# srisarya/nanopore-barcoding-ORC

Measured on AMD Instinct MI355X. Metric: Mreads/s two-round SP5×SP27 demux; % HBM roofline; 1/2/4/8 GPU, higher is better.
Workload: dtype u64

## Files before the change

nanopore-barcoding-orc_amd/csrc/dmx_device.h:

```cpp
#pragma once
#include <hip/hip_runtime.h>
#include <stdint.h>

namespace dmx {

constexpr int kMaxAdapters = 64;
constexpr int kMaxLen = 64;
constexpr int kRingSmall = 74;
constexpr int kRingLarge = 128;
constexpr int kScanBlock = 256;
constexpr int kResolveBlock = 64;

enum : uint8_t { kFront = 1, kBack = 2 };

struct DevAdapter {
    uint64_t peq[8];
    int8_t acc[72];
    int8_t pacc[72];
    uint8_t m;
    uint8_t k;
    uint8_t where;
    int8_t kk;
    uint8_t pad[4];
};
// ... 90 lines not shown

struct FTask {
    uint32_t item;
    uint32_t p0;
    uint16_t span;
    uint8_t hoff;
    uint8_t flags;
    uint32_t n, start, len;
    uint64_t off;
};
static_assert(sizeof(FTask) == 32, "FTask layout");

constexpr int kSuperNt = 4096;
constexpr int kCellGuardWords = 4;
constexpr int kCandStageCap = 128;

template <typename Rec, int CAP = kStageCap>
struct Stage {
    Rec* buf;
    uint32_t* cnt;
    uint32_t* base;
    Rec* g;
    uint32_t* gcount;
    uint32_t gcap;
    uint32_t* flags;
    uint32_t ovf;

    __device__ __forceinline__ void push(const Rec& r) const {
        const uint32_t i = atomicAdd(cnt, 1u);
        if (i < (uint32_t)CAP) {
            buf[i] = r;
            return;
        }
        const uint32_t gi = atomicAdd(gcount, 1u);
        if (gi < gcap) g[gi] = r;
        else atomicOr(flags, ovf);
    }
    __device__ __forceinline__ void flush() const {
        __syncthreads();
        const uint32_t n = min(*cnt, (uint32_t)CAP);
        if (threadIdx.x == 0) *base = n ? atomicAdd(gcount, n) : 0u;
        __syncthreads();
        const uint32_t b = *base;
        for (uint32_t i = threadIdx.x; i < n; i += blockDim.x) {
            if (b + i < gcap) g[b + i] = buf[i];
            else atomicOr(flags, ovf);
        }
        __syncthreads();
        if (threadIdx.x == 0) *cnt = 0;
        __syncthreads();
    }
};

__device__ __forceinline__ uint32_t stage_count(const uint32_t* c) {
    __syncthreads();
    const uint32_t v = *c;
    __syncthreads();
    return v;
}

struct ItemView {
    uint32_t read;
    uint32_t start;
    uint32_t len;
    uint8_t strand;
    uint8_t pad;
    int16_t only_adapter;
};

struct Cluster {
    uint32_t item;
    uint16_t sub;
    uint8_t lastcol;
    int8_t ub;
    uint32_t j1, j2;
};

struct Cand {
    uint32_t item;
    uint16_t sub;
    uint8_t iend;
    uint8_t cost;
    uint32_t j;
    uint32_t n, start, len;
    uint8_t strand, o, a, clean;
    uint64_t off;
};
static_assert(sizeof(Cand) == 40 && offsetof(Cand, off) == 32, "Cand layout");

struct Outcome {
    uint64_t key;
    int32_t origin;
    int32_t pad;
};

__host__ __device__ inline uint64_t make_key(int score, int o, int cost, int a, uint64_t t) {
    const int s = score < -128 ? -128 : score;
    return ((uint64_t)(127 - s) << 56) | ((uint64_t)o << 55) | ((uint64_t)cost << 48) |
           ((uint64_t)a << 40) | (t & ((1ull << 40) - 1));
}
__host__ __device__ inline int key_score(uint64_t k) { return 127 - (int)(k >> 56); }
__host__ __device__ inline int key_orient(uint64_t k) { return (int)((k >> 55) & 1); }
__host__ __device__ inline int key_cost(uint64_t k) { return (int)((k >> 48) & 127); }
__host__ __device__ inline int key_adapter(uint64_t k) { return (int)((k >> 40) & 255); }
__host__ __device__ inline uint64_t key_t(uint64_t k) { return k & ((1ull << 40) - 1); }

constexpr int kKeyPosBits = 40;
constexpr int kKeyDeltaBits = 4;
constexpr int kKeyDeltaBias = 8;
constexpr int kKeyDeltaMin = -kKeyDeltaBias;
constexpr int kBandMaxCost = 7;
static_assert(sizeof(uint32_t) * 8 + 1 <= kKeyPosBits - kKeyDeltaBits,
              "t = len + 1 + iend < 2^33 must fit above the delta code");
static_assert(kBandMaxCost < kKeyDeltaBias && kBandMaxCost + kKeyDeltaBias < (1 << kKeyDeltaBits),
              "|delta| <= cost <= 7 must fit the delta code");
__host__ __device__ inline uint64_t make_key_o(int score, int o, int cost, int a, uint64_t t,
                                               int delta) {
    return make_key(score, o, cost, a,
                    (t << kKeyDeltaBits) |
                        (uint64_t)((delta + kKeyDeltaBias) & ((1 << kKeyDeltaBits) - 1)));
}
__host__ __device__ inline uint64_t key_t_o(uint64_t k) { return key_t(k) >> kKeyDeltaBits; }
__host__ __device__ inline int key_delta(uint64_t k) {
    return (int)(k & ((1u << kKeyDeltaBits) - 1)) - kKeyDeltaBias;
}

enum EndType : uint8_t { kEndPrefix = 0, kEndFrontX = 1, kEndSuffix = 2, kEndBackX = 3 };
struct EndAdapter {
    uint64_t peq[4];
    int8_t acc[72];
    int8_t pacc[72];
    uint8_t m, k, type, orig;
    int8_t kk;
    uint8_t pad[3];
};
static_assert(sizeof(EndAdapter) == 184, "EndAdapter layout");
struct DevEnds {
    int32_t n;
    int32_t n_orient;
    int32_t n_sub;
    int32_t remap_on;
    uint8_t remap[kMaxAdapters];
    EndAdapter ad[kMaxAdapters];
};

enum BoundsBuf : uint32_t {
    kBufSeq = 1, kBufMask = 2, kBufSlot = 3, kBufItem = 4, kBufRes = 5, kBufCount = 6,
    kBufRead = 7, kBufLinked = 8, kBufCand = 9, kBufChop = 10, kBufPd = 11,
    kBufPaTrace = 12, kBufPaOps = 13, kBufGaCols = 14, kBufRdCols = 15, kBufRrCols = 16,
    kBufHistBins = 17, kBufRaCols = 18, kBufRaTable = 19, kBufRaBest = 20,
    kBufEndsSeq = 21, kBufEndsMask = 22, kBufEndsSlot = 23, kBufEndsItem = 24, kBufEndsRead = 25
};
enum BoundsKernel : int32_t {
    kKerFilter = 1, kKerVerify, kKerScreen, kKerScreen4, kKerWscan, kKerScan, kKerBand0,
    kKerBand1, kKerResolve, kKerSelect, kKerFin0, kKerFin1, kKerFin0L, kKerFin1L,
    kKerFin2L, kKerChop, kKerChopBig, kKerChopStart, kKerSelfTest, kKerPieces, kKerPairdist,
    kKerPairalign, kKerPairalignTb, kKerGroupalign, kKerGroupalignTb, kKerGroupalignMerge,
    kKerRowdist, kKerRowpair, kKerRowpairRc, kKerHithist, kKerRowassign,
    kKerRowassignDecide, kKerRowassignFinish, kKerEnds, kKerEndsOrigin, kKerEndsRemap,
    kKerChopViews
};
constexpr int kBoundsRec = 24;

struct Bounds {
#ifdef DMX_DEBUG_BOUNDS
    int64_t lo, hi;
    uint64_t slots, items, reads, counts, linked;
    uint64_t res, views, srcs;
    uint32_t* rec;
    int32_t kid;
#endif
};

__device__ __forceinline__ bool bchk(const Bounds& b, int64_t i, int64_t lo, int64_t hi,
                                     uint32_t buf) {
#ifdef DMX_DEBUG_BOUNDS
    if (i >= lo && i < hi) return true;
    atomicOr(b.rec + 3, 32u);
    if (atomicCAS(b.rec + kBoundsRec, 0u, (uint32_t)b.kid + 1u) == 0u) {
        b.rec[kBoundsRec + 1] = buf;
        b.rec[kBoundsRec + 2] = (uint32_t)(uint64_t)i;
        b.rec[kBoundsRec + 3] = (uint32_t)((uint64_t)i >> 32);
    }
    return false;
#else
    (void)b, (void)i, (void)lo, (void)hi, (void)buf;
    return true;
#endif
}
#ifdef DMX_DEBUG_BOUNDS
#define DMX_BOUND(bd, field, i, buf) bchk((bd), (int64_t)(i), 0, (int64_t)(bd).field, (buf))
#else
#define DMX_BOUND(bd, field, i, buf) true
#endif

constexpr int kGuardWords = 64;
constexpr int kGuardNt = 16 * kGuardWords;
constexpr int kMinOffset = 16;
constexpr int kMinTail = 64;
constexpr int kViewReachPre = 64;

struct Packed {
    const uint32_t* seq;
    const uint32_t* nmask;
    Bounds bd;
};
constexpr int kOffBits = 36;
constexpr uint64_t kOffMask = (1ull << kOffBits) - 1ull;

__device__ __forceinline__ uint32_t window32(const uint32_t* __restrict__ w, int64_t bitpos,
                                             const Bounds& bd, uint32_t buf) {
    const int64_t q = bitpos >> 5;
    const uint32_t sh = (uint32_t)bitpos & 31u;
#ifdef DMX_DEBUG_BOUNDS
    if (!bchk(bd, q, bd.lo, bd.hi - 1, buf)) return 0u;
#else
    (void)bd, (void)buf;
#endif
    uint64_t v;
    __builtin_memcpy(&v, w + q, 8);
    return (uint32_t)(v >> sh);
}
__device__ __forceinline__ uint32_t code32(const Packed& pk, int64_t g) {
    return window32(pk.seq, 2 * g, pk.bd, kBufSeq);
}
__device__ __forceinline__ uint32_t mask32(const Packed& pk, int64_t g) {
    return window32(pk.nmask, g, pk.bd, kBufMask);
}

__device__ __forceinline__ uint32_t rev_pairs(uint32_t w) {
    const uint32_t v = __brev(w);
    return ((v >> 1) & 0x55555555u) | ((v << 1) & 0xAAAAAAAAu);
}

__device__ __forceinline__ void fetch16(const Packed& pk, uint64_t off, uint32_t n,
                                        uint32_t strand, uint32_t start, uint32_t p,
                                        uint32_t& codes, uint32_t& nbits, bool load_mask = true) {
    if (strand == 0) {
        const int64_t g = (int64_t)off + start + p;
        codes = code32(pk, g);
        nbits = load_mask ? mask32(pk, g) & 0xFFFFu : 0u;
    } else {
        const int64_t b = (int64_t)off + (int64_t)n - 1 - start - (int64_t)p - 15;
        codes = ~rev_pairs(code32(pk, b));
        nbits = load_mask ? __brev(mask32(pk, b)) >> 16 : 0u;
    }
}

template <int HB>
__device__ __forceinline__ void myers_step_hw(uint32_t eql, uint32_t eqh, uint32_t& pvl,
                                              uint32_t& pvh, uint32_t& mvl, uint32_t& mvh, int& d,
                                              uint32_t hbit) {
    const uint32_t xvl = eql | mvl, xvh = eqh | mvh;
    uint32_t cy, cy2;
    const uint32_t sl = __builtin_addc(eql & pvl, pvl, 0u, &cy);
    const uint32_t sh = __builtin_addc(eqh & pvh, pvh, cy, &cy2);
    const uint32_t xhl = (sl ^ pvl) | eql, xhh = (sh ^ pvh) | eqh;
    const uint32_t phl = mvl | ~(xhl | pvl), phh = mvh | ~(xhh | pvh);
    const uint32_t mhl = pvl & xhl, mhh = pvh & xhh;
    uint32_t ps, ms;
    if constexpr (HB == 0) {
        ps = phl;
        ms = mhl;
    } else if constexpr (HB == 1) {
        ps = phh;
        ms = mhh;
    } else {
        ps = hbit >= 32 ? phh : phl;
        ms = hbit >= 32 ? mhh : mhl;
    }
    d += (int)__builtin_amdgcn_ubfe(ps, hbit & 31u, 1) +
         __builtin_amdgcn_sbfe((int)ms, hbit & 31u, 1);
    const uint32_t phh1 = __builtin_amdgcn_alignbit(phh, phl, 31), phl1 = phl << 1;
    const uint32_t mhh1 = __builtin_amdgcn_alignbit(mhh, mhl, 31), mhl1 = mhl << 1;
    pvl = mhl1 | ~(xvl | phl1);
    pvh = mhh1 | ~(xvh | phh1);
    mvl = phl1 & xvl;
    mvh = phh1 & xvh;
}

template <int HB = -1>
__device__ __forceinline__ void myers_step(uint64_t eq, uint64_t& pv, uint64_t& mv, int& d,
                                           uint32_t hbit) {
    uint32_t pvl = (uint32_t)pv, pvh = (uint32_t)(pv >> 32);
    uint32_t mvl = (uint32_t)mv, mvh = (uint32_t)(mv >> 32);
    myers_step_hw<HB>((uint32_t)eq, (uint32_t)(eq >> 32), pvl, pvh, mvl, mvh, d, hbit);
    pv = ((uint64_t)pvh << 32) | pvl;
    mv = ((uint64_t)mvh << 32) | mvl;
}

__device__ __forceinline__ void myers_step32(uint32_t eq, uint32_t& pv, uint32_t& mv, int& d,
                                             uint32_t hbit) {
    const uint32_t xv = eq | mv;
    const uint32_t xh = (((eq & pv) + pv) ^ pv) | eq;
    uint32_t ph = mv | ~(xh | pv);
    uint32_t mh = pv & xh;
    d += (int)__builtin_amdgcn_ubfe(ph, hbit, 1) + __builtin_amdgcn_sbfe((int)mh, hbit, 1);
    ph <<= 1;
    mh <<= 1;
    pv = mh | ~(xv | ph);
    mv = ph & xv;
}

__device__ __forceinline__ int col_cost(uint64_t pv, uint64_t mv, int i) {
    const uint64_t mask = i >= 64 ? ~0ull : ((1ull << i) - 1ull);
    return __popcll(pv & mask) - __popcll(mv & mask);
}

}
```

nanopore-barcoding-orc_amd/csrc/dmx_kernels.hip:

```cpp
#include <algorithm>
#include <cstring>
#include <memory>
#include <type_traits>
#include <utility>
#include <vector>

#include "dmx_device.h"
#include "dmx_internal.h"

namespace dmx {

struct RoundArgs {
    Packed pk;
    const uint64_t* offs;
    const uint32_t* lens;
    const DevPanel* panel;
    const ItemView* items;
    const uint32_t* n_items_dev;
    uint32_t n_items;
    int32_t T;
    int32_t per_task_slot;
    int32_t slot_div;
    Cluster* cl;
    Outcome* outc;
// ... 1753 lines not shown
                const bool reached = ps_emit(R, fbuf, fcnt, rr, item, o, tvo);
                ps_lastcol(R, wbuf, wcnt, last && !reached, item, o, tvo, rb);
            }
        }
    }
}

constexpr int kSbWords = kSuperNt / 16 + 8;

typedef __attribute__((address_space(1))) uint32_t gu32;
struct CellPtrs {
    gu32* p[4];
    __device__ __forceinline__ explicit CellPtrs(const RoundArgs& R) {
#pragma unroll
        for (int i = 0; i < 4; ++i) p[i] = sgpr_ptr(R.cells[i]);
    }
};

__device__ __forceinline__ void flat_check(const RoundArgs& R, const CellPtrs& cp,
                                           const PsTables& tb, uint64_t cw, uint64_t X,
                                           bool valid) {
    gu32* p1 = nullptr;
    uint32_t b1 = 0;
    if (valid) {
        const uint32_t kr = ps_key(tb, (uint32_t)(cw >> 6) & 0xFFFFu);
        const int64_t last = (int64_t)R.n_words * 16 - 1;
        const int e0 = (int)(kr & 0xFFFFu), e1 = e0 + (int)(kr >> 16);
        for (int e = e0; e < e1; ++e) {
            const uint64_t ev = tb.ent[e];
            const int len = (int)((ev >> 32) & 31u);
            const int off = (int)((ev >> 38) & 3u);
            const uint32_t msk = len >= 16 ? ~0u : ((1u << (2 * len)) - 1u);
            if (((uint32_t)(cw >> (2 * (3 - off))) & msk) != (uint32_t)ev) continue;
            const int tau = (int)((ev >> 37) & 1u);
            const int dlo = (int)((ev >> 40) & 255u) - 128;
            const int dhi = (int)((ev >> 48) & 255u) - 128;
            const int64_t x = (int64_t)X - off;
            int64_t nlo = tau ? x - dhi : x + len + dlo - 1;
            int64_t nhi = tau ? x - dlo : x + len + dhi - 1;
            nlo = nlo < 0 ? 0 : nlo;
            nhi = nhi > last ? last : nhi;
            if (nlo > nhi) continue;
            const int ci = 2 * (int)((ev >> 56) & 1u) + tau;
            gu32* cells = ci < 2 ? (ci == 0 ? cp.p[0] : cp.p[1]) : (ci == 2 ? cp.p[2] : cp.p[3]);
            for (int64_t c = nlo >> 4; c <= (nhi >> 4);) {
                const int64_t w = c >> 5;
                const int64_t cend = min(nhi >> 4, (w << 5) + 31);
                const uint32_t bits = (uint32_t)((((2ull << (cend - c)) - 1ull)) << (c & 31));
                if (!p1) {
                    p1 = cells + w;
                    b1 = bits;
                } else {
                    __hip_atomic_fetch_or(cells + w, bits, __ATOMIC_RELAXED, __HIP_MEMORY_SCOPE_AGENT);
                }
                c = cend + 1;
            }
        }
    }
    const uint64_t pa = (uint64_t)p1;
    const uint64_t pl = ((uint64_t)__shfl_up((uint32_t)(pa >> 32), 1u, 64) << 32) |
                        (uint64_t)__shfl_up((uint32_t)pa, 1u, 64);
    const uint32_t bl = __shfl_up(b1, 1u, 64);
    const bool dup = (threadIdx.x & 63u) != 0u && pl == pa && (bl & b1) == b1;
    if (p1 && !dup) {
        __hip_atomic_fetch_or(p1, b1, __ATOMIC_RELAXED, __HIP_MEMORY_SCOPE_AGENT);
    }
}

template <int S>
__global__ __launch_bounds__(kPScanBlock) void pscan_kernel(RoundArgs R) {
    static_assert(S == 1 || S == 2 || S == 4, "sampling stride: 64 positions per step");
    extern __shared__ __attribute__((aligned(16))) uint8_t s_dyn[];
    __shared__ __attribute__((aligned(16))) uint32_t s_sb[kPScanBlock / 64][kSbWords];
    __shared__ uint16_t s_q[kPScanBlock / 64][64];
    const PsTables tb = ps_load_tables(R.pieces, s_dyn);
    __syncthreads();
    const CellPtrs cp(R);
    const int lane = (int)(threadIdx.x & 63u);
    uint32_t* const sbw = s_sb[threadIdx.x >> 6];
    uint16_t* const q = s_q[threadIdx.x >> 6];
    const uint4* sp = reinterpret_cast<const uint4*>(R.pk.seq);
    const uint32_t nw = gridDim.x * (kPScanBlock / 64);
    for (uint32_t sb = blockIdx.x * (kPScanBlock / 64) + (threadIdx.x >> 6); sb < R.nsb; sb += nw) {
        const int64_t wd = (int64_t)sb * (kSuperNt / 16) + 4 * lane;
        const bool live = wd < (int64_t)R.n_words;
        uint4 c = {0u, 0u, 0u, 0u};
        if (live) c = sp[wd >> 2];
        uint32_t w0 = __shfl_up(c.w, 1u, 64), w5 = __shfl_down(c.x, 1u, 64);
        if (lane == 0) w0 = R.pk.seq[wd - 1];
        if (lane == 63) w5 = live ? R.pk.seq[wd + 4] : 0u;
        auto hits = ps_lookups<S>(tb.pr, w0, c.x, c.y, c.z, c.w, w5);
        using HitT = decltype(hits);
        if (!live) hits = 0;
        reinterpret_cast<uint4*>(sbw)[1 + lane] = c;
        if (lane == 0) sbw[3] = w0;
        if (lane == 63) {
            sbw[kSbWords - 4] = w5;
            sbw[kSbWords - 3] = 0u;
            sbw[kSbWords - 2] = 0u;
            sbw[kSbWords - 1] = 0u;
        }
        uint32_t total;
        uint32_t idx = wave_excl_scan((uint32_t)__popcll((unsigned long long)hits), total);
        const uint64_t C0 = (uint64_t)sb * kSuperNt;
        for (uint32_t base = 0; base < total; base += 64) {
            while (hits && idx < base + 64u) {
                const int qq = (int)__builtin_ctzll((unsigned long long)hits);
                hits &= hits - (HitT)1;
                q[idx - base] = (uint16_t)(lane * 64 + qq * S);
                ++idx;
            }
            __builtin_amdgcn_wave_barrier();
            const bool v = (uint32_t)lane < total - base;
            const uint32_t p = v ? q[lane] : 0u;
            const uint32_t t = p + 61u;
            const uint32_t wi = t >> 4, sh = 2u * (t & 15u);
            const uint64_t lo = ((uint64_t)sbw[wi + 1] << 32) | sbw[wi];
            const uint64_t cw = sh ? (lo >> sh) | ((uint64_t)sbw[wi + 2] << (64u - sh)) : lo;
            flat_check(R, cp, tb, cw, C0 + p, v);
            __builtin_amdgcn_wave_barrier();
        }
    }
}

__global__ __launch_bounds__(kScanBlock) void pcompact_kernel(RoundArgs R) {
    const DevPanel* P = R.panel;
    const DevPieces* Q = R.pieces;
    const uint32_t n_items = R.items ? *R.n_items_dev : R.n_items;
    const bool front = P->where == kFront;
    const int A = P->n_adapters;
    const int no = P->n_orient;
    const int W = P->scan_len + P->kf;
    const int SEG = kSegSpan - W;
    const int rb = kCleanHist ? P->clean_reach : 0;
    const int fr = Q->front_reach;
    const uint32_t wsh = wave_shard();
    FTask* const fbuf = R.ftask + wsh * R.ftask_scap;
    uint32_t* const fcnt = R.ftask_count + wsh * kShardStride;
    Window* const wbuf = R.win + wsh * R.win_scap;
    uint32_t* const wcnt = R.win_count + wsh * kShardStride;
    const uint32_t stride = gridDim.x * blockDim.x;
    const CellPtrs cp(R);
    const gu32* const cb0 = cp.p[2 * R.round];
    const gu32* const cb1 = cp.p[2 * R.round + 1];
    struct View {
        TaskView tv;
        int64_t p0nt = 0;
        int delta = 0, ncell = 0, l = 0;
        uint3 w = {0u, 0u, 0u};
    };
    const auto words = [&](const View& v, int k0, uint3& wv) __attribute__((always_inline)) {
        const int64_t c0 = v.p0nt >> 4;
        const int64_t cs = v.tv.strand ? c0 - k0 - 63 : c0 + k0;
        const gu32* cb = v.tv.strand ? cb1 : cb0;
        const int64_t w = k0 < v.ncell ? cs >> 5 : 0;
        wv.x = cb[w];
        wv.y = cb[w + 1];
        wv.z = cb[w + 2];
    };
    const auto prep = [&](uint32_t item, bool act, int o, View& v) __attribute__((always_inline)) {
        if (act) {
            task_view(R, item, o * A, A, v.tv);
            v.l = (int)v.tv.len;
        }
        v.p0nt = v.tv.strand ? (int64_t)v.tv.off + v.tv.n - 1 - v.tv.start
                             : (int64_t)v.tv.off + v.tv.start;
        v.delta = act ? (v.tv.strand ? 15 - (int)(v.p0nt & 15) : (int)(v.p0nt & 15)) : 0;
        v.ncell = act && v.l > 0 ? (v.l + v.delta + 15) >> 4 : 0;
        words(v, 0, v.w);
    };
    const auto run = [&](uint32_t item, bool act, int o, const View& v) __attribute__((always_inline)) {
        bool reached = false;
        uint3 cur = v.w;
        for (int k0 = 0; __ballot(k0 < v.ncell); k0 += 64) {
            uint3 nx = {0u, 0u, 0u};
            words(v, k0 + 64, nx);
            uint64_t m = 0;
            if (k0 < v.ncell) {
                const int64_t c0 = v.p0nt >> 4;
                const int64_t cs = v.tv.strand ? c0 - k0 - 63 : c0 + k0;
                const uint32_t sh = (uint32_t)(cs & 31);
                const uint64_t lo = ((uint64_t)cur.y << 32) | cur.x;
                const uint64_t x = sh ? (lo >> sh) | ((uint64_t)cur.z << (64 - sh)) : lo;
                m = v.tv.strand ? __builtin_bitreverse64(x) : x;
                if (front && k0 == 0)
                    m |= (fr + v.delta + 15) >> 4 >= 64 ? ~0ull
                                                        : ((1ull << ((fr + v.delta + 15) >> 4)) - 1ull);
                const int left = v.ncell - k0;
                if (left < 64) m &= (1ull << left) - 1ull;
                m |= ((m << 1) & (m >> 1)) | ((m << 1) & (m >> 2)) | ((m << 2) & (m >> 1));
            }
            PsRuns rr{m, k0, v.delta, v.l, W, SEG, 0, 0};
            reached |= ps_emit(R, fbuf, fcnt, rr, item, o, v.tv);
            cur = nx;
        }
        ps_lastcol(R, wbuf, wcnt, act && !front && !reached, item, o, v.tv, rb);
    };
    for (uint32_t i0 = blockIdx.x * blockDim.x; i0 < n_items; i0 += stride) {
        const uint32_t item = i0 + threadIdx.x;
        const bool act = item < n_items;
        View v0, v1;
        v0.tv.strand = v1.tv.strand = 0;
        const bool act1 = act && no > 1;
        prep(item, act, 0, v0);
        prep(item, act1, 1, v1);
        run(item, act, 0, v0);
        run(item, act1, 1, v1);
    }
}

__global__ __launch_bounds__(kScanBlock) __attribute__((amdgpu_waves_per_eu(DMX_FILTER_WAVES))) void ftask_kernel(RoundArgs R) {
    __shared__ uint32_t s_fpeq[8];
    __shared__ __attribute__((aligned(16))) int8_t s_thr[kScanBlock];
    __shared__ Window s_win[kScanBlock / 64][kWaveWinCap];
    __shared__ uint32_t s_wcnt[kScanBlock / 64];
    __shared__ uint32_t s_spre[kShards + 1];
    const DevPanel* P = R.panel;
    const int L = P->scan_len;
    const int kf = P->kf;
    if (threadIdx.x < 8) s_fpeq[threadIdx.x] = P->filter_peq[threadIdx.x];
    if (threadIdx.x < kScanBlock / 64) s_wcnt[threadIdx.x] = 0;
    {
        const int far0 = min((int)P->kf, (int)P->pf[71]);
        const int j = (int)threadIdx.x + 1;
        int t = -1;
        for (int d = 0; d <= far0; ++d)
            if (d <= (int)P->pf[min(j + d, 71)]) t = d;
        s_thr[threadIdx.x] = (int8_t)t;
    }
    ShardMap sm{s_spre, 0u};
    sm.load(R.ftask_count, R.ftask_scap);
    const uint32_t total = sm.total();
    const uint32_t wv = threadIdx.x >> 6;
    const uint32_t wsh = wave_shard();
    const WaveStage<Window, kWaveWinCap> st{s_win[wv], &s_wcnt[wv], R.win + wsh * R.win_scap,
                                            R.win_count + wsh * kShardStride, R.win_scap,
                                            R.flags, 4u};
    const bool front = P->where == kFront;
    const int kf_far = min(kf, (int)P->pf[71]);
    const uint32_t gap = (uint32_t)P->max_mk;
    const int rb = kCleanHist ? P->clean_reach : 0;
    const uint32_t pv_rows = L >= 32 ? ~0u : ~0u << (32 - L);
    for (uint32_t tb = blockIdx.x * kScanBlock; tb < total; tb += gridDim.x * kScanBlock) {
        const uint32_t ti = tb + threadIdx.x;
        if (ti < total) {
            const FTask ft = R.ftask[sm.phys(ti)];
            const int o = ft.flags & 1;
            const bool fresh = (ft.flags & 2) != 0;
            TaskView tv;
            tv.read = 0;
            tv.n = ft.n;
            tv.start = ft.start;
            tv.len = ft.len;
            tv.strand = (ft.flags >> 2) & 1u;
            tv.off = ft.off;
            tv.o = o;
            tv.a = 0;
            const uint32_t P0 = ft.p0;
            const uint32_t P1 = min(tv.len, P0 + (uint32_t)ft.span);
            const uint32_t hit_from = fresh ? 0u : P0 + ft.hoff;
            SegState S;
            S.pv = (fresh && front) ? 0u : pv_rows;
            S.mv = 0u;
            S.e = ((fresh && front) ? 0 : L) - (kf_far + 1);
            S.have = false;
            S.w1 = S.w2 = 0;
            S.wb = 255;
            filter_segment(R, tv, P0, P1, S, s_fpeq, s_thr, kf_far, gap, hit_from, rb, st,
                           ft.item, o);
            const uint32_t len = tv.len;
            if (!front && P1 == len) {
                if (S.have && len - S.w2 <= gap) {
                    st.push(make_window(ft.item, o, tv, S.w1, len, 1, S.wb,
                                        window_clean(S, S.w1, len, rb)));
                } else {
                    if (S.have)
                        st.push(make_window(ft.item, o, tv, S.w1, S.w2, 0, S.wb,
                                            window_clean(S, S.w1, S.w2, rb)));
                    st.push(make_window(ft.item, o, tv, len, len, 1, 255,
                                        window_clean(S, len, len, rb)));
                }
                S.have = false;
            }
            if (S.have)
                st.push(make_window(ft.item, o, tv, S.w1, S.w2, 0, S.wb,
                                    window_clean(S, S.w1, S.w2, rb)));
        }
        __builtin_amdgcn_wave_barrier();
        if (st.count() > kWaveWinCap / 2) st.flush();
    }
    __builtin_amdgcn_wave_barrier();
    st.flush();
}

#ifndef DMX_SORT_GROUP
#define DMX_SORT_GROUP 2048
#endif
constexpr int kSortGroup = DMX_SORT_GROUP;
constexpr int kSortBins = 64;
constexpr int kSortShift = 2;
static_assert(kSortGroup % kScanBlock == 0, "sort group");

#ifndef DMX_VERIFY_WAVES
#define DMX_VERIFY_WAVES 1
#endif
__global__ __launch_bounds__(kScanBlock) __attribute__((amdgpu_waves_per_eu(DMX_VERIFY_WAVES))) void verify_kernel(RoundArgs R) {
    __shared__ Window s_w[kStageCap];
    __shared__ uint32_t s_wc, s_wb;
    __shared__ int8_t s_pf[72];
    __shared__ uint32_t s_ppeq[8];
    if (threadIdx.x == 0) s_wc = 0;
    const DevPanel* P = R.panel;
    if (threadIdx.x < 72) s_pf[threadIdx.x] = P->pf[threadIdx.x];
    if (threadIdx.x < 8) s_ppeq[threadIdx.x] = P->pre_peq[threadIdx.x];
    __shared__ uint32_t s_spre[kShards + 1];
    ShardMap sm{s_spre, 0u};
    sm.load(R.win_count, R.win_scap);
    const uint32_t bsh = blockIdx.x & (uint32_t)(kShards - 1);
    const Stage<Window> st{s_w, &s_wc, &s_wb, R.win2 + bsh * R.win_scap,
                           R.win2_count + bsh * kShardStride,
                           R.win_scap, R.flags, 4u};
    const bool front = P->where == kFront;
    const int L = P->pre_len, kf = P->kf;
    const uint32_t total = sm.total();
    const bool sorted = front;
    __shared__ uint32_t s_ord[kSortGroup];
    __shared__ uint32_t s_bin[kSortBins];
    for (uint32_t gb = blockIdx.x * kSortGroup; gb < total; gb += gridDim.x * kSortGroup) {
      const uint32_t gn = min((uint32_t)kSortGroup, total - gb);
      if (sorted) {
        if (threadIdx.x < kSortBins) s_bin[threadIdx.x] = 0;
        __syncthreads();
        constexpr int PER = kSortGroup / kScanBlock;
        uint32_t key[PER], pos[PER];
#pragma unroll
        for (int e = 0; e < PER; ++e) {
            const uint32_t li = threadIdx.x + (uint32_t)e * kScanBlock;
            const Window* w = R.win + sm.phys(gb + min(li, gn - 1u));
            const int span = (int)w->j2 - (int)w->j1;
            key[e] = (uint32_t)min(max(span, 0) >> kSortShift, kSortBins - 1);
        }
#pragma unroll
        for (int e = 0; e < PER; ++e)
            if (threadIdx.x + (uint32_t)e * kScanBlock < gn) pos[e] = atomicAdd(&s_bin[key[e]], 1u);
        __syncthreads();
        if (threadIdx.x == 0) {
            uint32_t acc = 0;
            for (int b = 0; b < kSortBins; ++b) {
                const uint32_t c = s_bin[b];
                s_bin[b] = acc;
                acc += c;
            }
        }
        __syncthreads();
#pragma unroll
        for (int e = 0; e < PER; ++e) {
            const uint32_t li = threadIdx.x + (uint32_t)e * kScanBlock;
            if (li < gn) s_ord[s_bin[key[e]] + pos[e]] = li;
        }
        __syncthreads();
      }
      for (uint32_t sb = 0; sb < gn; sb += kScanBlock) {
        const uint32_t li = sb + threadIdx.x;
        if (li < gn) {
            Window w = R.win[sm.phys(gb + (sorted ? s_ord[li] : li))];
            const int len = (int)w.len;
            const bool rows_free = (front && (int)w.j1 <= P->max_mk) || w.bmin == 255;
            int lo = 1 << 30, hi = -1;
            if (!rows_free) {
                lo = (int)w.j1 - P->off_max - kf;
                hi = (int)w.j2 - P->off_min + kf;
            }
            const int end_lo = len - (P->m_max - 1 - L + kf);
            if (w.lastcol) {
                lo = min(lo, end_lo);
                hi = len;
            }
            bool keep = rows_free && w.bmin != 255;
            uint32_t info = 0;
            if (!keep && hi >= 0) {
                lo = max(lo, 0);
                hi = min(hi, len);
                TaskView tv;
                tv.read = 0;
                tv.n = w.n;
                tv.strand = w.strand & 1u;
                tv.start = w.start;
                tv.len = w.len;
                view_off(w.off, tv);
                tv.o = w.o;
                tv.a = 0;
                int js = lo - L - kf - 1;
                if (js < 0) js = 0;
                uint32_t pv = ~0u, mv = 0u;
                int d = L;
                int dmin_rows = 1 << 20, dmin_end = 1 << 20, dmin_near = 1 << 20;
                const int near_lo = len - (P->m_max - P->filter_len - L - 1) - kf;
                const uint32_t hbit = (uint32_t)(L - 1);
                const int rlo = w.bmin == 255 ? (1 << 30) : (int)w.j1 - P->off_max - kf;
                const int rhi = (int)w.j2 - P->off_min + kf;
                if (js == 0) {
                    if (rlo <= 0 && rhi >= 0) dmin_rows = L;
                    if (end_lo <= 0) dmin_end = L;
                    if (near_lo <= 0) dmin_near = L;
                }
                const int nst = (hi - js + 63) >> 6;
                ViewBlocks<false> vb;
                if (nst > 0) vb.init(R, tv, js);
                for (int st_i = 0; st_i < nst; ++st_i) {
                    uint32_t vc[4], vn[4];
                    vb.extract(vc, vn, st_i + 2 < nst);
#pragma unroll
                    for (int ch = 0; ch < 4; ++ch) {
                        const int p0 = js + 64 * st_i + 16 * ch;
                        const int cnt = min(16, hi - p0);
                        if (cnt <= 0) break;
                        const uint32_t codes = vc[ch], nb = vn[ch];
                        for (int q = 0; q < cnt; ++q) {
                            const uint32_t code = ((codes >> (2 * q)) & 3u) |
                                                  (((nb >> q) & 1u) << 2);
                            myers_step32(s_ppeq[code], pv, mv, d, hbit);
                            const int j = p0 + q + 1;
                            if (j >= rlo && j <= rhi) dmin_rows = min(dmin_rows, d);
                            if (j >= end_lo) dmin_end = min(dmin_end, d);
                            if (j >= near_lo) dmin_near = min(dmin_near, d);
                        }
                    }
                }
                if (!rows_free && (int)w.bmin + dmin_rows <= kf) keep = true;
                if (!rows_free) info = (uint32_t)min(dmin_rows, kf + 1);
                if (w.lastcol) {
                    if (dmin_end <= kf) keep = true;
                    info |= (uint32_t)min(dmin_end, kf + 1) << 8;
                    info |= (uint32_t)min(dmin_near, kf + 1) << 24;
                    int dd = 0;
                    bool pcell = false;
                    for (int i = 1; i <= L; ++i) {
                        dd += (int)((pv >> (i - 1)) & 1u) - (int)((mv >> (i - 1)) & 1u);
                        pcell |= dd <= (int)s_pf[i];
                    }
                    if (pcell || hi == 0) {
                        keep = true;
                        info |= 1u << 16;
                    }
                }
            }
            w.info = info;
            if (keep) st.push(w);
        }
        if (stage_count(&s_wc) > kStageCap / 2) st.flush();
      }
    }
    st.flush();
}


__device__ __forceinline__ Window make_task(Window w, uint32_t jlo, uint32_t jhi, bool lastcol,
                                            int a) {
    w.lastcol = lastcol ? 1 : 0;
    w.j1 = jlo;
    w.j2 = jhi;
    w.info = (uint32_t)a;
    return w;
}

__global__ __launch_bounds__(kScanBlock) void iscreen_kernel(RoundArgs R) {
    __shared__ uint32_t s_ipeq[kMaxAdapters * kIpeqStride];
    __shared__ int8_t s_acc[72 * kMaxAdapters];
    __shared__ Window s_task[kScanBlock / 64][kWaveWinCap];
    __shared__ uint32_t s_tc[kScanBlock / 64], s_nend;
    const DevPanel* P = R.panel;
    const int A = P->n_adapters;
    const int pl = P->pre_len, sl = P->filter_len, kf = P->kf;
    for (int x = threadIdx.x; x < 4 * A; x += blockDim.x) {
        const int c = x & 3, a = x >> 2;
        const int l = (int)P->ad[a].m - pl - sl;
        const uint64_t v = P->ad[a].peq[c] >> pl;
        s_ipeq[a * kIpeqStride + c] =
            l >= 32 ? (uint32_t)v
                    : ((uint32_t)(v & ((1ull << l) - 1ull)) << (32 - l)) | ((1u << (32 - l)) - 1u);
    }
    for (int x = threadIdx.x; x < 72 * A; x += blockDim.x) s_acc[x] = P->ad[x / 72].acc[x % 72];
    if (threadIdx.x < kScanBlock / 64) s_tc[threadIdx.x] = 0;
    if (threadIdx.x == 0) s_nend = 0;
    __shared__ uint32_t s_spre[kShards + 1];
    ShardMap sm{s_spre, 0u};
    sm.load(R.win2_count, R.win_scap);
    const uint32_t wv = threadIdx.x >> 6;
    const uint32_t wsh = wave_shard();
    const WaveStage<Window, kWaveWinCap> st{s_task[wv], &s_tc[wv], R.tasks + wsh * R.task_scap,
                                            R.task_count + wsh * kShardStride, R.task_scap,
                                            R.flags, 4u};
    const Window* wl = R.win2;
    const uint32_t nwin = sm.total();
    const uint32_t total = nwin * (uint32_t)A;
    const bool front = P->where == kFront;
    const int jsplit = front ? P->jsplit : 0;
    const int near_sh = front ? P->near_shared : -1;
    const bool pshared = P->pshared != 0;

    const uint32_t stride = gridDim.x * blockDim.x;
    for (uint32_t base = blockIdx.x * blockDim.x; base < total; base += stride) {
        const uint32_t t = base + threadIdx.x;
        if (t < total) {
            const uint32_t wi = t / (uint32_t)A;
            const int a = (int)(t - wi * (uint32_t)A);
            const Window w = wl[sm.phys(wi)];
            const DevAdapter& ad = P->ad[a];
            const int len = (int)w.len, j1 = (int)w.j1, j2 = (int)w.j2;
            const int l = (int)ad.m - pl - sl, kk = ad.kk;
            const int bm = w.bmin;
            const int dP = (int)(w.info & 255u), dPe = (int)((w.info >> 8) & 255u);
            const int dPn = (int)(w.info >> 24);
            const bool lastc = !front && w.lastcol;
            if (j1 < jsplit) {
                const int jh = min(j2, jsplit - 1);
                const int jl = a == 0 ? j1 : max(j1, near_sh + 1);
                if (jl <= jh) st.push(make_task(w, (uint32_t)jl, (uint32_t)jh, false, a));
            }
            const int jr = max(j1, jsplit);
            const int thr = kk - bm - dP;
            const bool rows = bm != 255 && jr <= j2 && thr >= 0;
            bool pass = lastc && (len == 0 || (((w.info >> 16) & 1u) && (a == 0 || !pshared)));
            bool by_end = true;
            const int thr_e = kk - dPe;
            if (!pass && (rows || lastc)) {
                const int xr_lo = jr - sl - kf, xr_hi = j2 - sl + kf;
                const int xe_lo = len - sl + 1 - kf;
                int xs = 1 << 30, xe = -1;
                if (rows) {
                    xs = xr_lo;
                    xe = min(xr_hi, len);
                }
                if (lastc) {
                    xs = min(xs, xe_lo);
                    xe = len;
                }
                int x1 = 1 << 30;
                if (rows) x1 = jr - l - sl - kf;
                if (lastc) x1 = min(x1, len - ((int)ad.m - 1 - pl) - kf);
                const int nch = (xe - x1 + 15) >> 4;
                const int jb = xe - 16 * nch;
                const int xrh = min(xr_hi, len);
                const char* ip = reinterpret_cast<const char*>(s_ipeq + a * kIpeqStride);
                const uint32_t rows_m = l >= 32 ? ~0u : ~0u << (32 - l);
                uint32_t pv = rows_m, mv = 0u;
                int d = l;
                TaskView tv;
                tv.read = 0;
                tv.n = w.n;
                tv.strand = w.strand & 1u;
                tv.start = w.start;
                tv.len = w.len;
                view_off(w.off, tv);
                tv.o = w.o;
                tv.a = a;
                uint32_t c0 = 0, n0 = 0, c1 = 0, n1 = 0;
                if (nch > 0) fetch16s<false>(R.pk, tv, jb, c0, n0);
                if (nch > 1) fetch16s<false>(R.pk, tv, jb + 16, c1, n1);
                for (int k = 0; k < nch && !pass; ++k) {
                    const int p0 = jb + 16 * k;
                    const uint32_t codes = c0, nb = n0;
                    c0 = c1;
                    n0 = n1;
                    if (k + 2 < nch) fetch16s<false>(R.pk, tv, p0 + 32, c1, n1);
                    const bool inR = rows && p0 + 16 >= xr_lo && p0 + 1 <= xrh;
                    const bool inE = lastc && p0 + 16 >= xe_lo;
                    const int tk = max(inR ? thr : -1, inE ? thr_e : -1);
                    const int qlo = min(inR ? xr_lo : (1 << 30), inE ? xe_lo : (1 << 30)) - p0 - 1;
                    uint32_t eq[16];
                    {
                        const uint32_t lo = spread_codes(codes, 0x0c010c00u);
                        const uint32_t hi = spread_codes(codes, 0x0c030c02u);
#pragma unroll
                        for (int q = 0; q < 16; ++q)
                            eq[q] = *reinterpret_cast<const uint32_t*>(
                                ip + __builtin_amdgcn_ubfe(q < 8 ? lo : hi, 4 * (q & 7), 4));
                    }
                    if (__builtin_amdgcn_ballot_w64(nb != 0u)) {
#pragma unroll
                        for (int q = 0; q < 16; ++q)
                            eq[q] &= ~((uint32_t)__builtin_amdgcn_sbfe((int)nb, q, 1) & rows_m);
                    }
                    int cm = 127;
                    if (__builtin_amdgcn_ballot_w64(qlo > 0) == 0) {
#pragma unroll
                        for (int q = 0; q < 16; ++q) {
                            myers_step_top(eq[q], pv, mv, d);
                            cm = min(cm, d);
                        }
                    } else {
#pragma unroll
                        for (int q = 0; q < 16; ++q) {
                            myers_step_top(eq[q], pv, mv, d);
                            cm = min(cm, q >= qlo ? d : 127);
                        }
                    }
                    pass = cm <= tk;
                    by_end = !inR;
                }
                if (lastc && !pass) {
                    int dd = 0;
                    const int sh = 32 - l;
                    for (int r = 1; r < l && !pass; ++r) {
                        dd += (int)((pv >> (sh + r - 1)) & 1u) - (int)((mv >> (sh + r - 1)) & 1u);
                        pass = dPn + dd <= (int)s_acc[72 * a + pl + r];
                    }
                }
            }
            if (pass) {
                st.push(make_task(w, (uint32_t)jr, (uint32_t)j2, lastc, a));
                if (by_end) atomicAdd(&s_nend, 1u);
            }
        }
        __builtin_amdgcn_wave_barrier();
        if (st.count() > kWaveWinCap / 2) st.flush();
    }
    __builtin_amdgcn_wave_barrier();
    st.flush();
    __syncthreads();
    if (threadIdx.x == 0 && s_nend) atomicAdd(&R.diag[3], s_nend);
}

typedef uint16_t u16x2 __attribute__((ext_vector_type(2)));
__device__ __forceinline__ u16x2 as_pk(uint32_t x) { return __builtin_bit_cast(u16x2, x); }
__device__ __forceinline__ uint32_t as_u32(u16x2 x) { return __builtin_bit_cast(uint32_t, x); }

__device__ __forceinline__ void myers_step_pk(uint32_t eq, uint32_t& pv, uint32_t& mv, u16x2& d) {
    const uint32_t xv = eq | mv;
    const uint32_t s = as_u32(as_pk(eq & pv) + as_pk(pv));
    const uint32_t ph = mv | ~(s | pv | eq);
    const uint32_t mh = pv & ((s ^ pv) | eq);
    d = d + (as_pk(ph) >> (uint16_t)15) - (as_pk(mh) >> (uint16_t)15);
    const uint32_t ph2 = as_u32(as_pk(ph) << (uint16_t)1);
    const uint32_t mh2 = as_u32(as_pk(mh) << (uint16_t)1);
    pv = mh2 | ~(xv | ph2);
    mv = ph2 & xv;
}

__device__ __forceinline__ void myers_step_pk_bare(uint32_t eq, uint32_t& pv, uint32_t& mv) {
    const uint32_t xv = eq | mv;
    const uint32_t s = as_u32(as_pk(eq & pv) + as_pk(pv));
    const uint32_t ph = mv | ~(s | pv | eq);
    const uint32_t mh = pv & ((s ^ pv) | eq);
    const uint32_t ph2 = as_u32(as_pk(ph) << (uint16_t)1);
    const uint32_t mh2 = as_u32(as_pk(mh) << (uint16_t)1);
    pv = mh2 | ~(xv | ph2);
    mv = ph2 & xv;
}

__device__ __forceinline__ u16x2 pk_cost_from_deltas(uint32_t pv, uint32_t mv) {
    const uint32_t lo = (uint32_t)__builtin_popcount(pv & 0xFFFFu) -
                        (uint32_t)__builtin_popcount(mv & 0xFFFFu);
    const uint32_t hi = (uint32_t)__builtin_popcount(pv >> 16) -
                        (uint32_t)__builtin_popcount(mv >> 16);
    return as_pk((lo & 0xFFFFu) | (hi << 16));
}

__device__ __forceinline__ uint32_t lds_off32(uint32_t f, uint32_t base) {
    uint32_t r;
    asm("v_lshl_add_u32 %0, %1, 5, %2" : "=v"(r) : "v"(f), "v"(base));
    return r;
}

#ifndef DMX_SCREEN_BARE
#define DMX_SCREEN_BARE 8
#endif
static_assert(DMX_SCREEN_BARE == 0 || DMX_SCREEN_BARE == 4 || DMX_SCREEN_BARE == 8 ||
              DMX_SCREEN_BARE == 16, "DMX_SCREEN_BARE: 0, 4, 8 or 16");

struct ScreenState {
    uint32_t pv0, mv0, pv1, mv1;
    u16x2 d0, d1;
    u16x2 m0, m1;
};

enum { kGroupBare = 0, kGroupCounted = 1, kGroupMasked = 2 };

template <int C0, int G, int KIND>
__device__ __forceinline__ void screen_cols(const char* qb, uint32_t lo, uint32_t hi, uint32_t q8,
                                            int qlo, ScreenState& s) {
#pragma unroll
    for (int c = C0; c < C0 + G; ++c) {
        const uint64_t e = *reinterpret_cast<const uint64_t*>(
            qb + lds_off32(__builtin_amdgcn_ubfe(c < 8 ? lo : hi, 4 * (c & 7), 4), q8));
        if constexpr (KIND == kGroupBare) {
            myers_step_pk_bare((uint32_t)e, s.pv0, s.mv0);
            myers_step_pk_bare((uint32_t)(e >> 32), s.pv1, s.mv1);
        } else {
            myers_step_pk((uint32_t)e, s.pv0, s.mv0, s.d0);
            myers_step_pk((uint32_t)(e >> 32), s.pv1, s.mv1, s.d1);
            if (KIND == kGroupCounted || c >= qlo) {
                s.m0 = __builtin_elementwise_min(s.m0, s.d0);
                s.m1 = __builtin_elementwise_min(s.m1, s.d1);
            }
        }
    }
}

template <int C0, int G>
__device__ __forceinline__ void screen_group(const char* qb, uint32_t lo, uint32_t hi, uint32_t q8,
                                             int qlo, ScreenState& s, bool& stale) {
    if (__builtin_amdgcn_ballot_w64(qlo < C0 + G) == 0) {
        screen_cols<C0, G, kGroupBare>(qb, lo, hi, q8, qlo, s);
        stale = true;
        return;
    }
    if (stale) {
        s.d0 = pk_cost_from_deltas(s.pv0, s.mv0);
        s.d1 = pk_cost_from_deltas(s.pv1, s.mv1);
        stale = false;
    }
    if (__builtin_amdgcn_ballot_w64(qlo > C0) == 0)
        screen_cols<C0, G, kGroupCounted>(qb, lo, hi, q8, qlo, s);
    else
        screen_cols<C0, G, kGroupMasked>(qb, lo, hi, q8, qlo, s);
}

template <int G>
__device__ __forceinline__ void screen_chunk(const char* qb, uint32_t lo, uint32_t hi, uint32_t q8,
                                             int qlo, ScreenState& s, bool& stale) {
    if constexpr (G == 16) {
        screen_group<0, 16>(qb, lo, hi, q8, qlo, s, stale);
    } else if constexpr (G == 8) {
        screen_group<0, 8>(qb, lo, hi, q8, qlo, s, stale);
        screen_group<8, 8>(qb, lo, hi, q8, qlo, s, stale);
    } else {
        screen_group<0, 4>(qb, lo, hi, q8, qlo, s, stale);
        screen_group<4, 4>(qb, lo, hi, q8, qlo, s, stale);
        screen_group<8, 4>(qb, lo, hi, q8, qlo, s, stale);
        screen_group<12, 4>(qb, lo, hi, q8, qlo, s, stale);
// ... 1861 lines not shown
```

Measured before the change: 365.9.

## Specialize verify Myers loop into wave-uniform bare/full/masked 8-column groups

Splits the per-column Myers verification loop into 8-column groups. When every lane in the wave is outside all tracked ranges, it runs a bare step that skips score tracking and recomputes the score lazily from popcounts. Otherwise it uses an unmasked min-tracking path when the ranges cover whole groups, and a masked path only at range edges. It also raises the verify kernel's waves-per-EU hint from 1 to 5, trading register budget for occupancy. The extra ballots and branches add code size and may cause divergence overhead.

```diff
diff --git a/nanopore-barcoding-orc_amd/csrc/dmx_device.h b/nanopore-barcoding-orc_amd/csrc/dmx_device.h
--- a/nanopore-barcoding-orc_amd/csrc/dmx_device.h
+++ b/nanopore-barcoding-orc_amd/csrc/dmx_device.h
@@ -416,6 +416,20 @@
     mv = ph & xv;
 }
 
+__device__ __forceinline__ void myers_step32_bare(uint32_t eq, uint32_t& pv, uint32_t& mv) {
+    const uint32_t xv = eq | mv;
+    const uint32_t xh = (((eq & pv) + pv) ^ pv) | eq;
+    const uint32_t ph = (mv | ~(xh | pv)) << 1;
+    const uint32_t mh = (pv & xh) << 1;
+    pv = mh | ~(xv | ph);
+    mv = ph & xv;
+}
+
+__device__ __forceinline__ int col_cost32(uint32_t pv, uint32_t mv, uint32_t hbit) {
+    const uint32_t mask = ~0u >> (31u - hbit);
+    return __popc(pv & mask) - __popc(mv & mask);
+}
+
 __device__ __forceinline__ int col_cost(uint64_t pv, uint64_t mv, int i) {
     const uint64_t mask = i >= 64 ? ~0ull : ((1ull << i) - 1ull);
     return __popcll(pv & mask) - __popcll(mv & mask);
diff --git a/nanopore-barcoding-orc_amd/csrc/dmx_kernels.hip b/nanopore-barcoding-orc_amd/csrc/dmx_kernels.hip
--- a/nanopore-barcoding-orc_amd/csrc/dmx_kernels.hip
+++ b/nanopore-barcoding-orc_amd/csrc/dmx_kernels.hip
@@ -2079,8 +2079,69 @@
 static_assert(kSortGroup % kScanBlock == 0, "sort group");
 
 #ifndef DMX_VERIFY_WAVES
-#define DMX_VERIFY_WAVES 1
+#define DMX_VERIFY_WAVES 5
 #endif
+
+struct VerifyState {
+    uint32_t pv, mv;
+    int d;
+    int m_rows, m_end, m_near;
+};
+
+enum { kVerBare = 0, kVerFull = 1, kVerMasked = 2 };
+
+template <int KIND>
+__device__ __forceinline__ void verify_cols(const uint32_t* ppeq, uint32_t codes, uint32_t nb,
+                                            int n, int ar, int br, int ae, int an, uint32_t hbit,
+                                            VerifyState& s) {
+    int gm = 1 << 20;
+#pragma unroll
+    for (int c = 0; c < 8; ++c) {
+        const uint32_t code = ((codes >> (2 * c)) & 3u) | (((nb >> c) & 1u) << 2);
+        if constexpr (KIND == kVerBare) {
+            myers_step32_bare(ppeq[code], s.pv, s.mv);
+        } else if constexpr (KIND == kVerFull) {
+            myers_step32(ppeq[code], s.pv, s.mv, s.d, hbit);
+            gm = min(gm, s.d);
+        } else {
+            if (c < n) {
+                myers_step32(ppeq[code], s.pv, s.mv, s.d, hbit);
+                if (c >= ar && c <= br) s.m_rows = min(s.m_rows, s.d);
+                if (c >= ae) s.m_end = min(s.m_end, s.d);
+                if (c >= an) s.m_near = min(s.m_near, s.d);
+            }
+        }
+    }
+    if constexpr (KIND == kVerFull) {
+        if (ar <= 0 && br >= 7) s.m_rows = min(s.m_rows, gm);
+        if (ae <= 0) s.m_end = min(s.m_end, gm);
+        if (an <= 0) s.m_near = min(s.m_near, gm);
+    }
+}
+
+__device__ __forceinline__ void verify_group(const uint32_t* ppeq, uint32_t codes, uint32_t nb,
+                                             int n, int j0, int rlo, int rhi, int end_lo,
+                                             int near_lo, uint32_t hbit, VerifyState& s,
+                                             bool& stale) {
+    const int ar = rlo - j0, br = rhi - j0, ae = end_lo - j0, an = near_lo - j0;
+    const bool whole = n >= 8;
+    const bool r_any = ar <= 7 && br >= 0, r_all = ar <= 0 && br >= 7;
+    const bool bare = whole && !r_any && ae > 7 && an > 7;
+    if (__builtin_amdgcn_ballot_w64(!bare) == 0) {
+        verify_cols<kVerBare>(ppeq, codes, nb, 8, ar, br, ae, an, hbit, s);
+        stale = true;
+        return;
+    }
+    if (stale) {
+        s.d = col_cost32(s.pv, s.mv, hbit);
+        stale = false;
+    }
+    const bool full = whole && r_any == r_all && (ae <= 0 || ae > 7) && (an <= 0 || an > 7);
+    if (__builtin_amdgcn_ballot_w64(!full) == 0)
+        verify_cols<kVerFull>(ppeq, codes, nb, 8, ar, br, ae, an, hbit, s);
+    else
+        verify_cols<kVerMasked>(ppeq, codes, nb, min(n, 8), ar, br, ae, an, hbit, s);
+}
 __global__ __launch_bounds__(kScanBlock) __attribute__((amdgpu_waves_per_eu(DMX_VERIFY_WAVES))) void verify_kernel(RoundArgs R) {
     __shared__ Window s_w[kStageCap];
     __shared__ uint32_t s_wc, s_wb;
@@ -2169,9 +2230,11 @@
                 tv.a = 0;
                 int js = lo - L - kf - 1;
                 if (js < 0) js = 0;
-                uint32_t pv = ~0u, mv = 0u;
-                int d = L;
-                int dmin_rows = 1 << 20, dmin_end = 1 << 20, dmin_near = 1 << 20;
+                VerifyState vs{~0u, 0u, L, 1 << 20, 1 << 20, 1 << 20};
+                bool stale = false;
+                int& dmin_rows = vs.m_rows;
+                int& dmin_end = vs.m_end;
+                int& dmin_near = vs.m_near;
                 const int near_lo = len - (P->m_max - P->filter_len - L - 1) - kf;
                 const uint32_t hbit = (uint32_t)(L - 1);
                 const int rlo = w.bmin == 255 ? (1 << 30) : (int)w.j1 - P->off_max - kf;
@@ -2190,20 +2253,17 @@
 #pragma unroll
                     for (int ch = 0; ch < 4; ++ch) {
                         const int p0 = js + 64 * st_i + 16 * ch;
-                        const int cnt = min(16, hi - p0);
+                        const int cnt = hi - p0;
                         if (cnt <= 0) break;
                         const uint32_t codes = vc[ch], nb = vn[ch];
-                        for (int q = 0; q < cnt; ++q) {
-                            const uint32_t code = ((codes >> (2 * q)) & 3u) |
-                                                  (((nb >> q) & 1u) << 2);
-                            myers_step32(s_ppeq[code], pv, mv, d, hbit);
-                            const int j = p0 + q + 1;
-                            if (j >= rlo && j <= rhi) dmin_rows = min(dmin_rows, d);
-                            if (j >= end_lo) dmin_end = min(dmin_end, d);
-                            if (j >= near_lo) dmin_near = min(dmin_near, d);
-                        }
+                        verify_group(s_ppeq, codes, nb, cnt, p0 + 1, rlo, rhi, end_lo, near_lo,
+                                     hbit, vs, stale);
+                        if (cnt > 8)
+                            verify_group(s_ppeq, codes >> 16, nb >> 8, cnt - 8, p0 + 9, rlo, rhi,
+                                         end_lo, near_lo, hbit, vs, stale);
                     }
                 }
+                const uint32_t pv = vs.pv, mv = vs.mv;
                 if (!rows_free && (int)w.bmin + dmin_rows <= kf) keep = true;
                 if (!rows_free) info = (uint32_t)min(dmin_rows, kf + 1);
                 if (w.lastcol) {
```

Result: no change. 367.3 (median of 2 runs) (+0.4%).
